# Sin7Y/olavm

Measured on AMD Instinct MI355X. Metric: goldilocks_ntt_throughput, higher is better.
Workload: dtype u64; 1 GPU; batched Goldilocks NTT (cfft::evaluate_poly), 94 cols x 2^22 rows per GPU, resident; log_n=22, columns_per_gpu=94, parallelism=columns sharded over 1 GPU(s), no collective, launch=single process

## Files before the change

olavm_amd/csrc/ntt2.hip:

```cpp
#include <hip/hip_runtime.h>

#include "device_ctx.h"
#include "gl.cuh"
#include "ntt2t.cuh"

namespace ola {

#ifndef NTT2_DEFAULT_GROUP_MB
#define NTT2_DEFAULT_GROUP_MB 0
#endif
#ifndef NTT2_STRIDED_COLS
#define NTT2_STRIDED_COLS 8
#endif

template <int K, bool INV>
__device__ __forceinline__ void dft_pow2(u64* x) {
#pragma unroll
    for (int i = K - 1; i >= 0; --i) {
#pragma unroll
        for (int j = 0; j < (1 << K); ++j) {
            if (j & (1 << i)) continue;
            const int e16 = (j & ((1 << i) - 1)) << (3 - i);
            const int t = ((INV ? 36 : 156) * e16) % 192;
            const u64 a = x[j], c = x[j + (1 << i)];
            x[j] = gl_add(a, c);
            const u64 d = (t >= 96) ? gl_sub(c, a) : gl_sub(a, c);
            x[j + (1 << i)] = gl_mul_pow2_sw(d, t % 96);
        }
    }
}

template <int R, int MODE, bool INV, int CB, bool PRE>
__device__ __forceinline__ void ntt2_pass_body(const Ntt2Params& p) {
    static_assert(!PRE || MODE == N2_STRIDED, "only the first (strided) pass of a coset transform pre-scales");
    static_assert(R >= 4 && R <= 8, "pass width");
    constexpr int K2 = R - 4;
    constexpr int D = 8 - R;
    constexpr int G2 = 1 << K2;
    constexpr int ROW = (1 << R) + 1;
    extern __shared__ __attribute__((aligned(16))) unsigned char smem_raw[];
    u64* lds = reinterpret_cast<u64*>(smem_raw);
    u64* tw1 = lds + ntt2_lds_elems<R, MODE>();

    const int tid = threadIdx.x;
    const u32 blk = blockIdx.x;
    const size_t col0 = (size_t)blockIdx.y * CB, coset = blockIdx.z;
    const int L = p.log_n, lo = p.lo;

    if (R > 4) {
        if (tid < (1 << R)) tw1[tid] = p.tw_r[tid];
    }

    auto pad1 = [](int e) -> int { return K2 >= 1 ? e + ((e >> (K2 + 4)) << 4) : e; };

    int uA, m_low, tA;
    if (MODE == N2_STRIDED) {
        uA = tid & 15;
        const int rest = tid >> 4;
        m_low = rest & ((1 << K2) - 1);
        tA = rest >> K2;
    } else {
        m_low = tid & ((1 << K2) - 1);
        uA = (tid >> K2) & 15;
        tA = tid >> R;
    }
    size_t a0;
    size_t jstride;
    size_t a0_uni = 0;
    u32 a0_lane = 0;
    {
        const u32 ntile = (blk << D) + tA;
        if (MODE == N2_STRIDED) {
            const u32 lowblks = 1u << (lo - 4);
            const u32 lb = ntile & (lowblks - 1), hi = ntile >> (lo - 4);
            a0 = ((size_t)hi << (lo + R)) + ((size_t)lb << 4) + ((size_t)m_low << lo) + uA;
            jstride = (size_t)1 << (lo + K2);
            const u32 ntile0 = blk << D;
            a0_uni = ((size_t)(ntile0 >> (lo - 4)) << (lo + R)) + ((size_t)(ntile0 & (lowblks - 1)) << 4);
            a0_lane = ((u32)tA << 4) + ((u32)m_low << lo) + (u32)uA;
        } else if (MODE == N2_BITREV_LAST) {
            a0 = ((((size_t)ntile << 4) + uA) << R) + m_low;
            jstride = (size_t)1 << K2;
        } else {
            const int ub = L - R - 4;
            const size_t row = ((size_t)rev_bits_c(uA, 4) << ub) + (ub ? bitrev32(ntile, ub) : 0);
            a0 = (row << R) + m_low;
            jstride = (size_t)1 << K2;
        }
    }
    const int uB = tid & 15, m_hi = tid >> 4;

    constexpr bool prescale = PRE;
    u64 up[PRE ? 16 : 1];
    if (prescale) {
        const u64 sb = two_level(p.sc_lo + coset * p.sc_coset_stride, p.sc_hi + coset * p.sc_coset_stride, p.sc_h, a0);
        const u64 st = p.sc_step[coset];
        u64 w = sb;
#pragma unroll
        for (int j = 0; j < 16; j++) {
            up[j] = w;
            if (j < 15) w = gl_mul(w, st);
        }
    }
    u64 wt[16];
    if (MODE == N2_STRIDED) {
        const u32 lowblks = 1u << (lo - 4);
#pragma unroll
        for (int t = 0; t < (1 << D); t++) {
            const u32 ntile = (blk << D) + t;
            const u64 low = ((u64)(ntile & (lowblks - 1)) << 4) + uB;
            u64 base = gl_mul(two_level(p.tw_lo, p.tw_hi, p.tw_h, low * (u64)rev_bits_c(m_hi & 15, 4)), p.post_scale);
            const u64 step = (K2 >= 1) ? two_level(p.tw_lo, p.tw_hi, p.tw_h, low << 4) : 1;
            u64 w = base;
#pragma unroll
            for (int k = 0; k < G2; k++) {
                wt[t * G2 + k] = w;
                if (k + 1 < G2) w = gl_mul(w, step);
            }
        }
    }

#pragma unroll 1
    for (int cc = 0; cc < CB; cc++) {
        const size_t col = col0 + cc;
        if (col >= p.ncols) break;
        const u64* __restrict__ in = p.in + col * p.in_col_stride + coset * p.in_coset_stride;
        u64* __restrict__ out = p.out + col * p.out_col_stride + coset * p.out_coset_stride;
        u32 zlane = 0;
        asm volatile("" : "+v"(zlane));

        {
            u64 x[16];
            if (MODE == N2_STRIDED) {
                const char* __restrict__ base = reinterpret_cast<const char*>(in + a0_uni);
                const u32 off = (a0_lane + zlane) * 8u;
#pragma unroll
                for (int j = 0; j < 16; j++) x[j] = gl_canon(*reinterpret_cast<const u64*>(base + j * jstride * 8 + off));
            } else {
#pragma unroll
                for (int j = 0; j < 16; j++) x[j] = gl_canon(in[a0 + j * jstride]);
            }
            if (prescale) {
#pragma unroll
                for (int j = 0; j < 16; j++) x[j] = gl_mul(x[j], up[j]);
            }
            dft_pow2<4, INV>(x);
            if (R > 4 && cc == 0) __syncthreads();
#pragma unroll
            for (int j = 0; j < 16; j++) {
                const int q1 = rev_bits_c(j, 4);
                u64 v = x[j];
                if (MODE == N2_STRIDED) {
                    if (R > 4 && q1 != 0) v = gl_mul(v, tw1[(q1 << K2) + m_low]);
                } else if (R > 4 && q1 != 0) {
                    const int idx = m_low * q1;
                    if (idx) v = gl_mul(v, tw1[idx]);
                }
                const int m = (j << K2) + m_low;
                if (MODE == N2_STRIDED) lds[pad1((((tA << R) + m) << 4) + uA)] = v;
                else lds[((tA << 4) + uA) * ROW + m] = v;
            }
        }
        __syncthreads();

        {
            u64 y[16];
#pragma unroll
            for (int t = 0; t < (1 << D); t++) {
#pragma unroll
                for (int j2 = 0; j2 < G2; j2++) {
                    const int m = (m_hi << K2) + j2;
                    y[t * G2 + j2] = (MODE == N2_STRIDED) ? lds[pad1((((t << R) + m) << 4) + uB)] : lds[((t << 4) + uB) * ROW + m];
                }
            }
#pragma unroll
            for (int t = 0; t < (1 << D); t++)
                if (K2 >= 1) dft_pow2<(K2 >= 1 ? K2 : 1), INV>(y + t * G2);
            if (MODE == N2_STRIDED) {
                const u32 lowblks = 1u << (lo - 4);
#pragma unroll
                for (int t = 0; t < (1 << D); t++) {
                    const u32 ntile = (blk << D) + t;
                    const u32 lb = ntile & (lowblks - 1), hi = ntile >> (lo - 4);
                    char* __restrict__ obase = reinterpret_cast<char*>(out + ((size_t)hi << (lo + R)) + ((size_t)lb << 4));
                    const u32 ooff = (((u32)m_hi << (K2 + lo)) + (u32)uB + zlane) * 8u;
#pragma unroll
                    for (int k = 0; k < G2; k++) {
                        const int j2 = rev_bits_c(k, K2);
                        *reinterpret_cast<u64*>(obase + ((size_t)j2 << (lo + 3)) + ooff) = gl_mul(y[t * G2 + j2], wt[t * G2 + k]);
                    }
                }
            } else if (MODE == N2_NATURAL_LAST) {
#pragma unroll
                for (int t = 0; t < (1 << D); t++) {
                    const u32 A = (blk << D) + t;
#pragma unroll
                    for (int j2 = 0; j2 < G2; j2++) {
                        const u32 q = ((u32)rev_bits_c(j2, K2) << 4) + (u32)rev_bits_c(m_hi & 15, 4);
                        out[((size_t)A << 4) + uB + ((size_t)q << (L - R))] = y[t * G2 + j2];
                    }
                }
            } else {
                __syncthreads();
#pragma unroll
                for (int t = 0; t < (1 << D); t++)
#pragma unroll
                    for (int j2 = 0; j2 < G2; j2++) lds[((t << 4) + uB) * ROW + (m_hi << K2) + j2] = y[t * G2 + j2];
                __syncthreads();
                const size_t b0 = (size_t)blk << 12;
#pragma unroll
                for (int k = 0; k < 16; k++) {
                    const int c = (k << 8) + tid;
                    out[b0 + c] = lds[(c >> R) * ROW + (c & ((1 << R) - 1))];
                }
            }
        }
        if (cc + 1 < CB) __syncthreads();
    }
}

template <int R, int MODE, bool INV, int CB, bool PRE>
__global__ __launch_bounds__(256) void ntt2_pass_kernel(Ntt2Params p) { ntt2_pass_body<R, MODE, INV, CB, PRE>(p); }
template <int R, int MODE, bool INV, int CB>
static void ntt2_launch_cb(const Ntt2Params& p0, size_t cols, size_t cosets, hipStream_t stream) {
    Ntt2Params p = p0;
    p.ncols = cols;
    const size_t lds_bytes = (size_t)(ntt2_lds_elems<R, MODE>() + (R > 4 ? (1 << R) : 0)) * 8;
    dim3 grid((unsigned)(((size_t)1 << p.log_n) >> 12), (unsigned)((cols + CB - 1) / CB), (unsigned)cosets);
    if (MODE == N2_STRIDED && p.sc_lo) hipLaunchKernelGGL((ntt2_pass_kernel<R, MODE, INV, CB, MODE == N2_STRIDED>), grid, dim3(256), lds_bytes, stream, p);
    else hipLaunchKernelGGL((ntt2_pass_kernel<R, MODE, INV, CB, false>), grid, dim3(256), lds_bytes, stream, p);
}
template <int R, int MODE, bool INV>
static void ntt2_launch(const Ntt2Params& p, size_t cols, size_t cosets, hipStream_t stream) {
    ntt2_launch_cb<R, MODE, INV, (MODE == N2_STRIDED ? NTT2_STRIDED_COLS : 1)>(p, cols, cosets, stream);
}
template <int MODE, bool INV>
static void ntt2_dispatch_r(int R, const Ntt2Params& p, size_t cols, size_t cosets, hipStream_t s) {
    switch (R) {
        case 4: ntt2_launch<4, MODE, INV>(p, cols, cosets, s); break;
        case 5: ntt2_launch<5, MODE, INV>(p, cols, cosets, s); break;
        case 6: ntt2_launch<6, MODE, INV>(p, cols, cosets, s); break;
        case 7: ntt2_launch<7, MODE, INV>(p, cols, cosets, s); break;
        default: ntt2_launch<8, MODE, INV>(p, cols, cosets, s); break;
    }
}
static void ntt2_dispatch(int R, int mode, bool inv, const Ntt2Params& p, size_t cols, size_t cosets, hipStream_t s) {
    if (mode == N2_STRIDED) { if (inv) ntt2_dispatch_r<N2_STRIDED, true>(R, p, cols, cosets, s); else ntt2_dispatch_r<N2_STRIDED, false>(R, p, cols, cosets, s); }
    else if (mode == N2_BITREV_LAST) { if (inv) ntt2_dispatch_r<N2_BITREV_LAST, true>(R, p, cols, cosets, s); else ntt2_dispatch_r<N2_BITREV_LAST, false>(R, p, cols, cosets, s); }
    else { if (inv) ntt2_dispatch_r<N2_NATURAL_LAST, true>(R, p, cols, cosets, s); else ntt2_dispatch_r<N2_NATURAL_LAST, false>(R, p, cols, cosets, s); }
}

static bool ntt2_tform() {
    static const bool v = [] { const char* e = getenv("OLA_NTT2_TFORM"); return !(e && atoi(e) == 0); }();
    return v;
}
template <int R, int MODE, bool INV, int LM>
static void ntt2t_launch(const Ntt2Params& p0, size_t cols, size_t cosets, hipStream_t stream) {
    constexpr int CB = NTT2_STRIDED_COLS;
    Ntt2Params p = p0;
    p.ncols = cols;
    const size_t lds_bytes = (size_t)ntt2_lds_elems<R, MODE>() * 8 + (R > 4 ? ((size_t)sizeof(TfTw) << R) : 0) + (LM == 1 ? ((size_t)8 << R) : 0);
    dim3 grid((unsigned)(((size_t)1 << p.log_n) >> 12), (unsigned)((cols + CB - 1) / CB), (unsigned)cosets);
    hipLaunchKernelGGL((ntt2t_pass_kernel<R, MODE, INV, CB, LM>), grid, dim3(256), lds_bytes, stream, p);
}
template <int MODE, bool INV, int LM>
static void ntt2t_dispatch_r(int R, const Ntt2Params& p, size_t cols, size_t cosets, hipStream_t s) {
    switch (R) {
        case 4: ntt2t_launch<4, MODE, INV, LM>(p, cols, cosets, s); break;
        case 5: ntt2t_launch<5, MODE, INV, LM>(p, cols, cosets, s); break;
        case 6: ntt2t_launch<6, MODE, INV, LM>(p, cols, cosets, s); break;
        case 7: ntt2t_launch<7, MODE, INV, LM>(p, cols, cosets, s); break;
        default: ntt2t_launch<8, MODE, INV, LM>(p, cols, cosets, s); break;
    }
}
template <bool INV>
static void ntt2t_dispatch_inv(int R, int mode, int lm, const Ntt2Params& p, size_t cols, size_t cosets, hipStream_t s) {
    if (mode == N2_STRIDED) {
        if (lm == 0) ntt2t_dispatch_r<N2_STRIDED, INV, 0>(R, p, cols, cosets, s);
        else ntt2t_dispatch_r<N2_STRIDED, INV, 1>(R, p, cols, cosets, s);
    } else if (mode == N2_BITREV_LAST) ntt2t_dispatch_r<N2_BITREV_LAST, INV, 2>(R, p, cols, cosets, s);
    else ntt2t_dispatch_r<N2_NATURAL_LAST, INV, 2>(R, p, cols, cosets, s);
}
static void ntt2t_dispatch(int R, int mode, bool inv, int lm, const Ntt2Params& p, size_t cols, size_t cosets, hipStream_t s) {
    if (inv) ntt2t_dispatch_inv<true>(R, mode, lm, p, cols, cosets, s);
    else ntt2t_dispatch_inv<false>(R, mode, lm, p, cols, cosets, s);
}
static void ntt2t_dispatch_timed(NttTables& t, int R, int mode, bool inv, int lm, const Ntt2Params& p, size_t cols, size_t cosets, hipStream_t s) {
    if (!t.pass_timing || t.pass_recs.size() >= 4096) { ntt2t_dispatch(R, mode, inv, lm, p, cols, cosets, s); return; }
    NttTables::PassRec r{R, mode, lm, inv, ((size_t)1 << p.log_n) * cols * cosets, nullptr, nullptr};
    HIP_CHECK(hipEventCreate(&r.a));
    HIP_CHECK(hipEventCreate(&r.b));
    HIP_CHECK(hipEventRecord(r.a, s));
    ntt2t_dispatch(R, mode, inv, lm, p, cols, cosets, s);
    HIP_CHECK(hipEventRecord(r.b, s));
    t.pass_recs.push_back(r);
}

static const u64* get_round_table(NttTables& t, int R, int inverse) {
    auto key = std::make_pair(200 + R, inverse);
    auto it = t.small.find(key);
    if (it != t.small.end()) return it->second;
    const std::vector<u64> full = powers(root_for(R, inverse), (size_t)1 << R);
    std::vector<u64> v;
    for (int q1 = 0; q1 < 16; q1++)
        for (int m = 0; m < (1 << (R - 4)); m++) v.push_back(full[(size_t)m * q1]);
    return t.small[key] = upload(t.ctx, v);
}

static const u64* get_full_small(NttTables& t, int R, int inverse) {
    auto key = std::make_pair(100 + R, inverse);
    auto it = t.small.find(key);
    if (it != t.small.end()) return it->second;
    std::vector<u64> v = powers(root_for(R, inverse), (size_t)1 << R);
    return t.small[key] = upload(t.ctx, v);
}

static const u64* get_coset_steps(NttTables& t, int log_n, int rate_bits, int e, u64 single_shift) {
    std::vector<u64> v;
    for (u64 s : coset_shifts(log_n, rate_bits, single_shift)) v.push_back(gl_pow(s, (u64)1 << e));
    return upload(t.ctx, v);
}

static const u64* get_coset_pows(NttTables& t, int log_n, int rate_bits, int lo, int R, u64 single_shift) {
    std::vector<u64> v;
    for (u64 sc : coset_shifts(log_n, rate_bits, single_shift)) {
        const std::vector<u64> pw = powers(gl_pow(sc, (u64)1 << lo), (size_t)1 << R);
        v.insert(v.end(), pw.begin(), pw.end());
    }
    return upload(t.ctx, v);
}

static void ntt2_run_group(NttTables& t, const u64* in, size_t in_col_stride, u64* out, size_t out_col_stride, u64* scratch,
                           size_t scratch_col_stride, int L, size_t cols, bool inverse, bool natural_out, int sc_rate_bits, u64 sc_shift,
                           size_t cosets, size_t out_coset_stride, size_t coset_first) {
    hipStream_t stream = t.ctx->stream;
    const int P = (L + 7) / 8;
    std::vector<int> Rs = split_even(L, P);
    std::reverse(Rs.begin(), Rs.end());
    const u64 final_scale = inverse ? gl_inv(((u64)1 << L) % GL_P) : 1;
    u64* work = natural_out ? scratch : out;
    const size_t work_col_stride = natural_out ? scratch_col_stride : out_col_stride;
    const size_t work_coset_stride = natural_out ? 0 : out_coset_stride;

    const u64* cur_in = in;
    size_t cur_in_stride = in_col_stride, cur_in_coset = 0;
    int lo = L;
    if (ntt2_tform() && L <= 28) {
        for (int i = 0; i < P; i++) {
            const int R = Rs[i];
            lo -= R;
            const bool last = (i == P - 1);
            Ntt2Params p = {};
            p.log_n = L; p.lo = lo;
            p.tw_r = get_round_table(t, R, inverse);
            p.post_scale = last ? final_scale : 1;
            p.in = cur_in; p.in_col_stride = cur_in_stride; p.in_coset_stride = cur_in_coset;
            if (i > 0) {
                TwoLevel tw = get_two(t, L - lo, inverse);
                p.tw_lo = tw.lo; p.tw_hi = tw.hi; p.tw_h = tw.h;
            }
            if (sc_rate_bits != -2) {
                const auto skey = std::make_tuple(L, sc_rate_bits, 1000 + lo * 16 + R, sc_rate_bits >= 0 ? (u64)0 : sc_shift);
                auto st = t.coset_steps.find(skey);
                if (st == t.coset_steps.end()) st = t.coset_steps.emplace(skey, get_coset_pows(t, L, sc_rate_bits, lo, R, sc_shift)).first;
                p.sc_pow = st->second + (coset_first << R);
            }
            const int lm = last ? 2 : ((i > 0 || p.sc_pow) ? 1 : 0);
            if (!last) {
                p.out = work; p.out_col_stride = work_col_stride; p.out_coset_stride = work_coset_stride;
                if (lo - 4 < 8 - R) throw OlaError(-7, "ntt2: pass split leaves a strided pass with lo + R < 12");
                ntt2t_dispatch_timed(t, R, N2_STRIDED, inverse, lm, p, cols, cosets, stream);
                cur_in = work; cur_in_stride = work_col_stride; cur_in_coset = work_coset_stride;
            } else {
                p.out = out; p.out_col_stride = out_col_stride; p.out_coset_stride = out_coset_stride;
                ntt2t_dispatch_timed(t, R, natural_out ? N2_NATURAL_LAST : N2_BITREV_LAST, inverse, 2, p, cols, cosets, stream);
            }
        }
        return;
    }
    for (int i = 0; i < P; i++) {
        const int R = Rs[i];
        lo -= R;
        const bool last = (i == P - 1);
        Ntt2Params p = {};
        p.log_n = L; p.lo = lo;
        p.tw_r = last ? get_full_small(t, R, inverse) : get_round_table(t, R, inverse);
        p.post_scale = 1;
        p.in = cur_in; p.in_col_stride = cur_in_stride; p.in_coset_stride = cur_in_coset;
        if (!last) {
            TwoLevel tw = get_two(t, lo + R, inverse);
            p.tw_lo = tw.lo; p.tw_hi = tw.hi; p.tw_h = tw.h;
            if (i == P - 2) p.post_scale = final_scale;
            p.out = work; p.out_col_stride = work_col_stride; p.out_coset_stride = work_coset_stride;
            if (i == 0 && sc_rate_bits != -2) {
                TwoLevel sc;
                size_t stride = 0;
                if (sc_rate_bits >= 0) sc = get_coset(t, L, sc_rate_bits, &stride);
                else sc = get_shift(t, L, sc_shift);
                p.sc_lo = sc.lo + coset_first * stride; p.sc_hi = sc.hi + coset_first * stride; p.sc_h = sc.h; p.sc_coset_stride = stride;
                {
                    const auto skey = std::make_tuple(L, sc_rate_bits, lo + R - 4, sc_rate_bits >= 0 ? (u64)0 : sc_shift);
                    auto st = t.coset_steps.find(skey);
                    if (st == t.coset_steps.end()) st = t.coset_steps.emplace(skey, get_coset_steps(t, L, sc_rate_bits, lo + R - 4, sc_shift)).first;
                    p.sc_step = st->second + coset_first;
                }
            }
            if (lo - 4 < 8 - R) throw OlaError(-7, "ntt2: pass split leaves a strided pass with lo + R < 12");
            ntt2_dispatch(R, N2_STRIDED, inverse, p, cols, cosets, stream);
            cur_in = work; cur_in_stride = work_col_stride; cur_in_coset = work_coset_stride;
        } else {
            p.out = out; p.out_col_stride = out_col_stride; p.out_coset_stride = out_coset_stride;
            ntt2_dispatch(R, natural_out ? N2_NATURAL_LAST : N2_BITREV_LAST, inverse, p, cols, cosets, stream);
        }
    }
}

static size_t ntt2_group_bytes() {
    const char* e = getenv("OLA_NTT2_GROUP_MB");
    return e ? (size_t)atol(e) << 20 : (size_t)NTT2_DEFAULT_GROUP_MB << 20;
}

void ntt2_run(NttTables& t, const u64* in, size_t in_col_stride, u64* out, size_t out_col_stride, u64* scratch,
              size_t scratch_col_stride, int L, size_t cols, bool inverse, bool natural_out, int sc_rate_bits, u64 sc_shift,
              size_t cosets, size_t out_coset_stride, size_t coset_first) {
    if (cols == 0) return;
    const size_t budget = ntt2_group_bytes(), col_bytes = ((size_t)8 << L) * (natural_out ? 2 : 1);
    size_t gc = cols, gk = cosets;
    if (budget && L >= 18 && col_bytes * cols * cosets > budget) {
        const size_t unit = NTT2_STRIDED_COLS;
        gk = 1;
        gc = std::max<size_t>(unit, budget / col_bytes / unit * unit);
        if (gc >= cols) { gc = cols; gk = std::max<size_t>(1, std::min(cosets, budget / (col_bytes * cols))); }
    }
    for (size_t c0 = 0; c0 < cols; c0 += gc) {
        const size_t nc = std::min(gc, cols - c0);
        for (size_t k0 = 0; k0 < cosets; k0 += gk) {
            const size_t nk = std::min(gk, cosets - k0);
            ntt2_run_group(t, in + c0 * in_col_stride, in_col_stride, out + c0 * out_col_stride + k0 * out_coset_stride, out_col_stride,
                           scratch ? scratch + c0 * scratch_col_stride : nullptr, scratch_col_stride, L, nc, inverse, natural_out,
                           sc_rate_bits, sc_shift, nk, out_coset_stride, coset_first + k0);
        }
    }
}

}
```

olavm_amd/csrc/ntt2t.cuh:

```cuda
#pragma once
#include <hip/hip_runtime.h>

#include "gl.cuh"
#include "tform.cuh"

namespace ola {

enum { N2_STRIDED = 0, N2_BITREV_LAST = 1, N2_NATURAL_LAST = 2 };

struct Ntt2Params {
    const u64* in;
    u64* out;
    size_t in_col_stride, out_col_stride, in_coset_stride, out_coset_stride;
    int log_n;
    size_t ncols;
    int lo;
    const u64* tw_r;
    const u64* tw_lo;
    const u64* tw_hi;
    int tw_h;
    u64 post_scale;
    const u64* sc_lo;
    const u64* sc_hi;
    int sc_h;
    size_t sc_coset_stride;
    const u64* sc_step;
    const u64* sc_pow;
};

__device__ __forceinline__ constexpr int rev_bits_c(int x, int bits) {
    int r = 0;
    for (int i = 0; i < bits; i++) r |= ((x >> i) & 1) << (bits - 1 - i);
    return r;
}

__device__ __forceinline__ u64 two_level(const u64* __restrict__ lo, const u64* __restrict__ hi, int h, u64 e) {
    return gl_mul(lo[e & (((u64)1 << h) - 1)], hi[e >> h]);
}

template <int R, int MODE>
constexpr int ntt2_lds_elems() {
    constexpr int K2 = R - 4;
    if (MODE == N2_STRIDED) return 4096 + (K2 >= 1 ? 16 * (4096 >> (K2 + 4)) : 0);
    return (1 << (8 - R)) * 16 * ((1 << R) + 1);
}

template <int R, int MODE, bool INV, int CB, int LM>
__device__ __forceinline__ void ntt2t_pass_body(const Ntt2Params& p) {
    static_assert(R >= 4 && R <= 8, "pass width");
    static_assert((LM == 2) == (MODE != N2_STRIDED), "strided passes keep their multipliers in LDS, closing passes in registers");
    constexpr int K2 = R - 4;
    constexpr int D = 8 - R;
    constexpr int G2 = 1 << K2;
    constexpr int ROW = (1 << R) + 1;
    extern __shared__ __attribute__((aligned(16))) unsigned char smem_raw[];
    u64* lds = reinterpret_cast<u64*>(smem_raw);
    TfTw* tw1 = reinterpret_cast<TfTw*>(lds + ntt2_lds_elems<R, MODE>());
    u64* lmtab = reinterpret_cast<u64*>(tw1 + (R > 4 ? (1 << R) : 0));

    const int tid = threadIdx.x;
    const u32 blk = blockIdx.x;
    const size_t col0 = (size_t)blockIdx.y * CB, coset = blockIdx.z;
    const int L = p.log_n, lo = p.lo;

    if (R > 4) {
        if (tid < (1 << R)) tw1[tid] = tf_split_u64(p.tw_r[tid]);
    }

    auto pad1 = [](int e) -> int { return K2 >= 1 ? e + ((e >> (K2 + 4)) << 4) : e; };

    int uA, m_low, tA;
    if (MODE == N2_STRIDED) {
        uA = tid & 15;
        const int rest = tid >> 4;
        m_low = rest & ((1 << K2) - 1);
        tA = rest >> K2;
    } else {
        m_low = tid & ((1 << K2) - 1);
        uA = (tid >> K2) & 15;
        tA = tid >> R;
    }
    size_t a0, jstride;
    size_t a0_uni = 0;
    u32 a0_lane = 0;
    {
        const u32 ntile = (blk << D) + tA;
        if (MODE == N2_STRIDED) {
            const u32 lowblks = 1u << (lo - 4);
            const u32 lb = ntile & (lowblks - 1), hi = ntile >> (lo - 4);
            a0 = ((size_t)hi << (lo + R)) + ((size_t)lb << 4) + ((size_t)m_low << lo) + uA;
            jstride = (size_t)1 << (lo + K2);
            const u32 ntile0 = blk << D;
            a0_uni = ((size_t)(ntile0 >> (lo - 4)) << (lo + R)) + ((size_t)(ntile0 & (lowblks - 1)) << 4);
            a0_lane = ((u32)tA << 4) + ((u32)m_low << lo) + (u32)uA;
        } else if (MODE == N2_BITREV_LAST) {
            a0 = ((((size_t)ntile << 4) + uA) << R) + m_low;
            jstride = (size_t)1 << K2;
        } else {
            const int ub = L - R - 4;
            const size_t row = ((size_t)rev_bits_c(uA, 4) << ub) + (ub ? bitrev32(ntile, ub) : 0);
            a0 = (row << R) + m_low;
            jstride = (size_t)1 << K2;
        }
    }
    const int uB = tid & 15, m_hi = tid >> 4;

    const int HB = L - lo - R;
    u64 wl[LM == 2 ? 16 : 1];
    if (LM == 1) {
        if (tid < (1 << R)) {
            const u32 hi = (blk << D) >> (lo - 4);
            const u64 K = HB ? bitrev32(hi, HB) : 0;
            u64 v = 1;
            if (p.tw_lo) v = two_level(p.tw_lo, p.tw_hi, p.tw_h, K * (u64)tid);
            if (p.sc_pow) v = p.tw_lo ? gl_mul(v, p.sc_pow[(coset << R) + tid]) : p.sc_pow[(coset << R) + tid];
            lmtab[tid] = v;
        }
    } else if (LM == 2) {
        const u64 K = bitrev32((u32)(a0 >> R), HB);
        u64 base = gl_mul(two_level(p.tw_lo, p.tw_hi, p.tw_h, K * (u64)m_low), p.post_scale);
        u64 step = two_level(p.tw_lo, p.tw_hi, p.tw_h, K << K2);
        if (p.sc_pow) {
            base = gl_mul(base, p.sc_pow[(coset << R) + m_low]);
            step = gl_mul(step, p.sc_pow[(coset << R) + (1 << K2)]);
        }
        u64 w = base;
#pragma unroll
        for (int j = 0; j < 16; j++) {
            wl[j] = w;
            if (j < 15) w = gl_mul(w, step);
        }
    }

    if (LM == 1 || R > 4) __syncthreads();

#pragma unroll 1
    for (int cc = 0; cc < CB; cc++) {
        const size_t col = col0 + cc;
        if (col >= p.ncols) break;
        const u64* __restrict__ in = p.in + col * p.in_col_stride + coset * p.in_coset_stride;
        u64* __restrict__ out = p.out + col * p.out_col_stride + coset * p.out_coset_stride;
        u32 zlane = 0;
        asm volatile("" : "+v"(zlane));

        T4 y[16];
        {
            T4 x[16];
            {
                u64 raw[16];
                if (MODE == N2_STRIDED) {
                    const char* __restrict__ base = reinterpret_cast<const char*>(in + a0_uni);
                    const u32 off = (a0_lane + zlane) * 8u;
#pragma unroll
                    for (int j = 0; j < 16; j++) raw[j] = *reinterpret_cast<const u64*>(base + j * jstride * 8 + off);
                } else {
#pragma unroll
                    for (int j = 0; j < 16; j++) raw[j] = in[a0 + j * jstride];
                }
#pragma unroll
                for (int j = 0; j < 16; j++) {
                    if (LM) {
                        u64 plo, phi;
                        mul_wide(raw[j], LM == 1 ? lmtab[(j << K2) + m_low] : wl[j], plo, phi);
                        x[j] = tf_from_u128(plo, phi);
                    } else {
                        x[j] = tf_from_u64(raw[j]);
                    }
                }
            }
            tf_dft<4, INV>(x);
            if (R > 4) {
#pragma unroll
                for (int j = 0; j < 16; j++) {
                    const int q1 = rev_bits_c(j, 4);
                    if (q1 != 0) x[j] = tf_mul(x[j], tw1[(q1 << K2) + m_low]);
                    else x[j] = tf_norm(x[j]);
                }
            }
#pragma unroll
            for (int h = 0; h < 2; h++) {
                if (h == 1) __syncthreads();
#pragma unroll
                for (int j = 0; j < 16; j++) {
                    const int m = (j << K2) + m_low;
                    const u64 v = (u64)(u32)x[j].v[2 * h] | ((u64)(u32)x[j].v[2 * h + 1] << 32);
                    if (MODE == N2_STRIDED) lds[pad1((((tA << R) + m) << 4) + uA)] = v;
                    else lds[((tA << 4) + uA) * ROW + m] = v;
                }
                __syncthreads();
#pragma unroll
                for (int t = 0; t < (1 << D); t++) {
#pragma unroll
                    for (int j2 = 0; j2 < G2; j2++) {
                        const int m = (m_hi << K2) + j2;
                        const u64 v = (MODE == N2_STRIDED) ? lds[pad1((((t << R) + m) << 4) + uB)] : lds[((t << 4) + uB) * ROW + m];
                        y[t * G2 + j2].v[2 * h] = (i32)(u32)v;
                        y[t * G2 + j2].v[2 * h + 1] = (i32)(u32)(v >> 32);
                    }
                }
            }
        }

#pragma unroll
        for (int t = 0; t < (1 << D); t++)
            if (K2 >= 1) tf_dft<(K2 >= 1 ? K2 : 1), INV>(y + t * G2);
        if (MODE == N2_STRIDED) {
            const u32 lowblks = 1u << (lo - 4);
#pragma unroll
            for (int t = 0; t < (1 << D); t++) {
                const u32 ntile = (blk << D) + t;
                const u32 lb = ntile & (lowblks - 1), hi = ntile >> (lo - 4);
                char* __restrict__ obase = reinterpret_cast<char*>(out + ((size_t)hi << (lo + R)) + ((size_t)lb << 4));
                const u32 ooff = (((u32)m_hi << (K2 + lo)) + (u32)uB + zlane) * 8u;
#pragma unroll
                for (int j2 = 0; j2 < G2; j2++)
                    *reinterpret_cast<u64*>(obase + ((size_t)j2 << (lo + 3)) + ooff) = tf_to_u64<false>(y[t * G2 + j2]);
            }
        } else if (MODE == N2_NATURAL_LAST) {
#pragma unroll
            for (int t = 0; t < (1 << D); t++) {
                const u32 A = (blk << D) + t;
                const u32 ooff = ((((u32)rev_bits_c(m_hi & 15, 4)) << (L - R)) + (u32)uB + zlane) * 8u;
#pragma unroll
                for (int j2 = 0; j2 < G2; j2++) {
                    char* __restrict__ obase = reinterpret_cast<char*>(out + ((size_t)A << 4) + ((size_t)rev_bits_c(j2, K2) << (L - R + 4)));
                    *reinterpret_cast<u64*>(obase + ooff) = tf_to_u64<true>(y[t * G2 + j2]);
                }
            }
        } else {
            __syncthreads();
#pragma unroll
            for (int t = 0; t < (1 << D); t++)
#pragma unroll
                for (int j2 = 0; j2 < G2; j2++) lds[((t << 4) + uB) * ROW + (m_hi << K2) + j2] = tf_to_u64<true>(y[t * G2 + j2]);
            __syncthreads();
            const size_t b0 = (size_t)blk << 12;
#pragma unroll
            for (int k = 0; k < 16; k++) {
                const int c = (k << 8) + tid;
                out[b0 + c] = lds[(c >> R) * ROW + (c & ((1 << R) - 1))];
            }
        }
        if (cc + 1 < CB) __syncthreads();
    }
}

template <int R, int MODE, bool INV, int CB, int LM>
__global__ __launch_bounds__(256, (MODE == N2_STRIDED ? 4 : 1)) void ntt2t_pass_kernel(Ntt2Params p) { ntt2t_pass_body<R, MODE, INV, CB, LM>(p); }

}
```

olavm_amd/csrc/tform.cuh:

```cuda
#pragma once
#include "gl.cuh"

namespace ola {

typedef int i32;
typedef long long i64;

GL_HD u32 tf_alignbit(u32 hi, u32 lo, int s) {
#if defined(__HIP_DEVICE_COMPILE__)
    return __builtin_amdgcn_alignbit(hi, lo, s);
#else
    return (u32)((((u64)hi << 32) | lo) >> s);
#endif
}

struct T4 {
    i32 v[4];
};
struct TfTw {
    i32 w0, w1, w2, pad;
};

GL_HD void tf_pin(T4& y) {
#if defined(__HIP_DEVICE_COMPILE__)
    asm("" : "+v"(y.v[0]), "+v"(y.v[1]), "+v"(y.v[2]), "+v"(y.v[3]));
#else
    (void)y;
#endif
}

GL_HD TfTw tf_split_u64(u64 w) {
    const u32 lo = (u32)w, hi = (u32)(w >> 32);
    TfTw t;
    t.w0 = (i32)(lo & 0xFFFFFFu);
    t.w1 = (i32)(((lo >> 24) | (hi << 8)) & 0xFFFFFFu);
    t.w2 = (i32)(hi >> 16);
    t.pad = 0;
    return t;
}

GL_HD T4 tf_from_u64(u64 x) {
    const u32 lo = (u32)x, hi = (u32)(x >> 32);
    T4 r;
    r.v[0] = (i32)(lo & 0xFFFFFFu);
    r.v[1] = (i32)(tf_alignbit(hi, lo, 24) & 0xFFFFFFu);
    r.v[2] = (i32)(hi >> 16);
    r.v[3] = 0;
    return r;
}
GL_HD T4 tf_from_u128(u64 lo, u64 hi) {
    const u32 l0 = (u32)lo, l1 = (u32)(lo >> 32), h0 = (u32)hi, h1 = (u32)(hi >> 32);
    T4 r;
    r.v[0] = (i32)(l0 & 0xFFFFFFu) - (i32)(h1 & 0xFFFFFFu);
    r.v[1] = (i32)(tf_alignbit(l1, l0, 24) & 0xFFFFFFu) - (i32)(h1 >> 24);
    r.v[2] = (i32)(tf_alignbit(h0, l1, 16) & 0xFFFFFFu);
    r.v[3] = (i32)(h0 >> 8);
    return r;
}

template <bool CANON>
GL_HD u64 tf_to_u64(const T4& x) {
    u32 u0 = (u32)x.v[0] + 0x80000080u, u1 = (u32)x.v[1] + 0x7FFFFF80u;
    u32 u2 = (u32)x.v[2] + 0x7FFFFF80u, u3 = (u32)x.v[3] + 0x7FFFFF80u;
    const u32 n1 = u1 & 0xFFFFFFu;
    u2 += u1 >> 24;
    const u32 n2 = u2 & 0xFFFFFFu;
    u3 += u2 >> 24;
    const u32 n3 = u3 & 0xFFFFFFu;
    u0 -= u3 >> 24;
    const u64 A = (u64)n1 * 0x1000000ull + u0;
    const u32 chi = (n3 << 8) | (n2 >> 16);
    const u32 d16 = n2 << 16;
#if defined(OLA_GL_ASM)
    const u32 a_lo = (u32)A, a_hi = (u32)(A >> 32);
    u32 hi1, e1, e2;
    u64 cA, cB, t2;
    asm("v_add_co_u32_e64 %0, %1, %2, %3" : "=v"(hi1), "=s"(cA) : "v"(a_hi), "v"(d16));
    asm("s_nop 1\n\tv_cndmask_b32_e64 %0, 0, -1, %1" : "=v"(e1) : "s"(cA));
    const u64 lo = (((u64)hi1 << 32) | a_lo) + e1;
    asm("v_mad_u64_u32 %0, %1, %2, -1, %3" : "=v"(t2), "=s"(cB) : "v"(chi), "v"(lo));
    if (!CANON) {
        asm("s_nop 1\n\tv_cndmask_b32_e64 %0, 0, -1, %1" : "=v"(e2) : "s"(cB));
        return t2 + e2;
    }
    const u32 tl = (u32)t2, th = (u32)(t2 >> 32);
    u32 ul, uh, r0, r1;
    u64 c1, c2, m;
    asm("v_add_co_u32_e64 %0, %1, -1, %2" : "=v"(ul), "=s"(c1) : "v"(tl));
    asm("s_nop 1\n\tv_addc_co_u32_e64 %0, %1, 0, %2, %3" : "=v"(uh), "=s"(c2) : "v"(th), "s"(c1));
    asm("s_nop 1\n\ts_or_b64 %2, %3, %4\n\tv_cndmask_b32_e64 %0, %5, %6, %2\n\tv_cndmask_b32_e64 %1, %7, %8, %2"
        : "=&v"(r0), "=&v"(r1), "=&s"(m) : "s"(cB), "s"(c2), "v"(tl), "v"(ul), "v"(th), "v"(uh) : "scc");
    return ((u64)r1 << 32) | r0;
#else
    u64 lo = A + ((u64)d16 << 32);
    if (lo < A) lo += GL_EPS;
    const u64 prod = (u64)chi * GL_EPS;
    u64 t2 = lo + prod;
    if (t2 < lo) t2 += GL_EPS;
    return CANON ? gl_canon(t2) : t2;
#endif
}

GL_HD T4 tf_add(const T4& a, const T4& b) {
    T4 r;
#pragma unroll
    for (int i = 0; i < 4; i++) r.v[i] = a.v[i] + b.v[i];
    return r;
}

GL_HD T4 tf_norm(const T4& x) {
    const i32 mask = 0xFFFFFF;
    T4 y;
    y.v[0] = (x.v[0] & mask) - (x.v[3] >> 24);
    y.v[1] = (x.v[1] & mask) + (x.v[0] >> 24);
    y.v[2] = (x.v[2] & mask) + (x.v[1] >> 24);
    y.v[3] = (x.v[3] & mask) + (x.v[2] >> 24);
    return y;
}

template <int S>
GL_HD T4 tf_sub_mul_pow2(const T4& a, const T4& b) {
    static_assert(S >= 0 && S < 192, "shift out of range");
    constexpr int q8 = S / 24, r = S % 24, q = q8 & 3;
    constexpr bool neg = q8 >= 4;
    T4 o;
    if (r == 0) {
#pragma unroll
        for (int i = 0; i < 4; i++) {
            const bool flip = neg != (i + q >= 4);
            o.v[(i + q) & 3] = flip ? (b.v[i] - a.v[i]) : (a.v[i] - b.v[i]);
        }
    } else {
        constexpr int k = 24 - r;
        const i32 mask = (i32)((1 << k) - 1);
        T4 d;
#pragma unroll
        for (int i = 0; i < 4; i++) d.v[i] = neg ? (b.v[i] - a.v[i]) : (a.v[i] - b.v[i]);
        T4 y;
        y.v[0] = ((d.v[0] & mask) << r) - (d.v[3] >> k);
        y.v[1] = ((d.v[1] & mask) << r) + (d.v[0] >> k);
        y.v[2] = ((d.v[2] & mask) << r) + (d.v[1] >> k);
        y.v[3] = ((d.v[3] & mask) << r) + (d.v[2] >> k);
#pragma unroll
        for (int i = 0; i < 4; i++) {
            if (i + q >= 4) o.v[(i + q) & 3] = -y.v[i];
            else o.v[i + q] = y.v[i];
        }
    }
    return o;
}

GL_HD T4 tf_mul(const T4& x_in, const TfTw& w) {
    T4 x = x_in;
    tf_pin(x);
    const i32 w0 = w.w0, w1 = w.w1, w2 = w.w2;
    const i32 n2 = -x.v[2], n3 = -x.v[3];
    i64 z[4];
    z[0] = (i64)x.v[0] * w0 + (i64)n3 * w1 + (i64)n2 * w2;
    z[1] = (i64)x.v[0] * w1 + (i64)x.v[1] * w0 + (i64)n3 * w2;
    z[2] = (i64)x.v[0] * w2 + (i64)x.v[1] * w1 + (i64)x.v[2] * w0;
    z[3] = (i64)x.v[1] * w2 + (i64)x.v[2] * w1 + (i64)x.v[3] * w0;
    i32 l[4], m[4], h[4];
#pragma unroll
    for (int k = 0; k < 4; k++) {
        const u32 lo = (u32)(u64)z[k];
        const i32 hi = (i32)(z[k] >> 32);
        l[k] = (i32)(lo & 0xFFFFFFu);
        m[k] = (i32)(tf_alignbit((u32)hi, lo, 24) & 0xFFFFFFu);
        h[k] = hi >> 16;
    }
    T4 y;
    y.v[0] = l[0] - m[3] - h[2];
    y.v[1] = l[1] + m[0] - h[3];
    y.v[2] = l[2] + m[1] + h[0];
    y.v[3] = l[3] + m[2] + h[1];
    tf_pin(y);
    return y;
}

GL_HD constexpr int tf_root_exp(int k, bool inv) {
    int e = 39;
    for (int i = k; i < 6; i++) e = (2 * e) % 192;
    return inv ? (192 - e) % 192 : e;
}

template <int K, bool INV>
GL_HD void tf_dft(T4* x) {
    static_assert(K >= 0 && K <= 4, "radix");
#pragma unroll
    for (int i = K - 1; i >= 0; --i) {
#pragma unroll
        for (int j = 0; j < (1 << K); ++j) {
            if (j & (1 << i)) continue;
            const int e = (j & ((1 << i) - 1)) << (3 - i);
            const int s = (tf_root_exp(4, INV) * e) % 192;
            const T4 a = x[j], b = x[j + (1 << i)];
            x[j] = tf_add(a, b);
            switch (s) {
#define OLA_TF_CASE(S) case S: x[j + (1 << i)] = tf_sub_mul_pow2<S>(a, b); break;
                OLA_TF_CASE(0) OLA_TF_CASE(12) OLA_TF_CASE(24) OLA_TF_CASE(36) OLA_TF_CASE(48) OLA_TF_CASE(60) OLA_TF_CASE(72) OLA_TF_CASE(84)
                OLA_TF_CASE(96) OLA_TF_CASE(108) OLA_TF_CASE(120) OLA_TF_CASE(132) OLA_TF_CASE(144) OLA_TF_CASE(156) OLA_TF_CASE(168)
                OLA_TF_CASE(180)
#undef OLA_TF_CASE
                default: break;
            }
        }
    }
}

}
```

Measured before the change: 1510 GB/s.

## Close Goldilocks NTT with a 6-bit pass using shift-only twiddles

```diff
diff --git a/olavm_amd/csrc/ntt2.hip b/olavm_amd/csrc/ntt2.hip
--- a/olavm_amd/csrc/ntt2.hip
+++ b/olavm_amd/csrc/ntt2.hip
@@ -254,12 +254,32 @@
     static const bool v = [] { const char* e = getenv("OLA_NTT2_TFORM"); return !(e && atoi(e) == 0); }();
     return v;
 }
+static int ntt2_close6() {
+    static const int v = [] { const char* e = getenv("OLA_NTT2_CLOSE6"); return e ? atoi(e) : 1; }();
+    return v;
+}
+static std::vector<int> ntt2t_widths(int L) {
+    const int P = (L + 7) / 8;
+    std::vector<int> even = split_even(L, P);
+    std::reverse(even.begin(), even.end());
+    if (ntt2_close6() == 0 || (P < 3 && ntt2_close6() != 2)) return even;
+    std::vector<int> v = split_even(L - 6, P - 1);
+    std::reverse(v.begin(), v.end());
+    int lo = L;
+    for (int R : v) {
+        lo -= R;
+        if (R < 4 || R > 8 || lo - 4 < 8 - R) return even;
+    }
+    v.push_back(6);
+    return v;
+}
 template <int R, int MODE, bool INV, int LM>
 static void ntt2t_launch(const Ntt2Params& p0, size_t cols, size_t cosets, hipStream_t stream) {
     constexpr int CB = NTT2_STRIDED_COLS;
     Ntt2Params p = p0;
     p.ncols = cols;
-    const size_t lds_bytes = (size_t)ntt2_lds_elems<R, MODE>() * 8 + (R > 4 ? ((size_t)sizeof(TfTw) << R) : 0) + (LM == 1 ? ((size_t)8 << R) : 0);
+    constexpr bool tw1 = R > 4 && !(R == 6 && MODE != N2_STRIDED);
+    const size_t lds_bytes = (size_t)ntt2_lds_elems<R, MODE>() * 8 + (tw1 ? ((size_t)sizeof(TfTw) << R) : 0) + (LM == 1 ? ((size_t)8 << R) : 0);
     dim3 grid((unsigned)(((size_t)1 << p.log_n) >> 12), (unsigned)((cols + CB - 1) / CB), (unsigned)cosets);
     hipLaunchKernelGGL((ntt2t_pass_kernel<R, MODE, INV, CB, LM>), grid, dim3(256), lds_bytes, stream, p);
 }
@@ -346,6 +366,7 @@
     size_t cur_in_stride = in_col_stride, cur_in_coset = 0;
     int lo = L;
     if (ntt2_tform() && L <= 28) {
+        Rs = ntt2t_widths(L);
         for (int i = 0; i < P; i++) {
             const int R = Rs[i];
             lo -= R;
diff --git a/olavm_amd/csrc/ntt2t.cuh b/olavm_amd/csrc/ntt2t.cuh
--- a/olavm_amd/csrc/ntt2t.cuh
+++ b/olavm_amd/csrc/ntt2t.cuh
@@ -45,6 +45,12 @@
     return (1 << (8 - R)) * 16 * ((1 << R) + 1);
 }
 
+template <int ML, bool INV>
+__device__ __forceinline__ void ntt2t_close6_put(const T4* x, int h, u64* dst) {
+    if (h == 0) tf_round6_pair<ML, INV, 0>(x, dst, 4);
+    else tf_round6_pair<ML, INV, 1>(x, dst, 4);
+}
+
 template <int R, int MODE, bool INV, int CB, int LM>
 __device__ __forceinline__ void ntt2t_pass_body(const Ntt2Params& p) {
     static_assert(R >= 4 && R <= 8, "pass width");
@@ -53,6 +59,7 @@
     constexpr int D = 8 - R;
     constexpr int G2 = 1 << K2;
     constexpr int ROW = (1 << R) + 1;
+    constexpr bool CLOSE6 = (R == 6 && MODE != N2_STRIDED);
     extern __shared__ __attribute__((aligned(16))) unsigned char smem_raw[];
     u64* lds = reinterpret_cast<u64*>(smem_raw);
     TfTw* tw1 = reinterpret_cast<TfTw*>(lds + ntt2_lds_elems<R, MODE>());
@@ -63,7 +70,7 @@
     const size_t col0 = (size_t)blockIdx.y * CB, coset = blockIdx.z;
     const int L = p.log_n, lo = p.lo;
 
-    if (R > 4) {
+    if (R > 4 && !CLOSE6) {
         if (tid < (1 << R)) tw1[tid] = tf_split_u64(p.tw_r[tid]);
     }
 
@@ -75,6 +82,10 @@
         const int rest = tid >> 4;
         m_low = rest & ((1 << K2) - 1);
         tA = rest >> K2;
+    } else if (CLOSE6) {
+        m_low = __builtin_amdgcn_readfirstlane(tid >> 6);
+        uA = tid & 15;
+        tA = (tid >> 4) & 3;
     } else {
         m_low = tid & ((1 << K2) - 1);
         uA = (tid >> K2) & 15;
@@ -132,7 +143,7 @@
         }
     }
 
-    if (LM == 1 || R > 4) __syncthreads();
+    if (LM == 1 || (R > 4 && !CLOSE6)) __syncthreads();
 
 #pragma unroll 1
     for (int cc = 0; cc < CB; cc++) {
@@ -153,6 +164,22 @@
                     const u32 off = (a0_lane + zlane) * 8u;
 #pragma unroll
                     for (int j = 0; j < 16; j++) raw[j] = *reinterpret_cast<const u64*>(base + j * jstride * 8 + off);
+                } else if (CLOSE6) {
+                    const u32 wv = (u32)m_low, ln = (u32)tid & 63u;
+                    const u32 ntile = (blk << D) + wv;
+                    const u32 off = (ln + zlane) * 8u;
+#pragma unroll
+                    for (int k = 0; k < 16; k++) {
+                        size_t row;
+                        if (MODE == N2_BITREV_LAST) row = ((size_t)ntile << 4) + k;
+                        else row = ((size_t)rev_bits_c(k, 4) << (L - R - 4)) + bitrev32(ntile, L - R - 4);
+                        raw[k] = *reinterpret_cast<const u64*>(reinterpret_cast<const char*>(in + (row << R)) + off);
+                    }
+#pragma unroll
+                    for (int k = 0; k < 16; k++) lds[((wv << 4) + k) * ROW + ln] = raw[k];
+                    __syncthreads();
+#pragma unroll
+                    for (int j = 0; j < 16; j++) raw[j] = lds[((tA << 4) + uA) * ROW + (j << K2) + m_low];
                 } else {
 #pragma unroll
                     for (int j = 0; j < 16; j++) raw[j] = in[a0 + j * jstride];
@@ -169,7 +196,11 @@
                 }
             }
             tf_dft<4, INV>(x);
-            if (R > 4) {
+            if (CLOSE6) {
+#pragma unroll
+                for (int j = 0; j < 16; j++) tf_pin(x[j]);
+            }
+            if (R > 4 && !CLOSE6) {
 #pragma unroll
                 for (int j = 0; j < 16; j++) {
                     const int q1 = rev_bits_c(j, 4);
@@ -179,9 +210,18 @@
             }
 #pragma unroll
             for (int h = 0; h < 2; h++) {
-                if (h == 1) __syncthreads();
-#pragma unroll
-                for (int j = 0; j < 16; j++) {
+                if (h == 1 || CLOSE6) __syncthreads();
+                if (CLOSE6) {
+                    u64* dst = lds + ((tA << 4) + uA) * ROW + m_low;
+                    switch (m_low) {
+                        case 0: ntt2t_close6_put<0, INV>(x, h, dst); break;
+                        case 1: ntt2t_close6_put<1, INV>(x, h, dst); break;
+                        case 2: ntt2t_close6_put<2, INV>(x, h, dst); break;
+                        default: ntt2t_close6_put<3, INV>(x, h, dst); break;
+                    }
+                }
+#pragma unroll
+                for (int j = 0; j < 16 && !CLOSE6; j++) {
                     const int m = (j << K2) + m_low;
                     const u64 v = (u64)(u32)x[j].v[2 * h] | ((u64)(u32)x[j].v[2 * h + 1] << 32);
                     if (MODE == N2_STRIDED) lds[pad1((((tA << R) + m) << 4) + uA)] = v;
diff --git a/olavm_amd/csrc/tform.cuh b/olavm_amd/csrc/tform.cuh
--- a/olavm_amd/csrc/tform.cuh
+++ b/olavm_amd/csrc/tform.cuh
@@ -14,8 +14,14 @@
 #endif
 }
 
+#if defined(OLA_TF_LIMB)
+typedef OLA_TF_LIMB tf_limb;
+#else
+typedef i32 tf_limb;
+#endif
+
 struct T4 {
-    i32 v[4];
+    tf_limb v[4];
 };
 struct TfTw {
     i32 w0, w1, w2, pad;
@@ -150,11 +156,36 @@
     return o;
 }
 
+template <int S, int T>
+GL_HD tf_limb tf_mul_pow2_limb(const T4& x) {
+    static_assert(S >= 0 && S < 192 && T >= 0 && T < 4, "shift or limb out of range");
+    constexpr int q8 = S / 24, r = S % 24, q = q8 & 3;
+    constexpr int i = (T - q) & 3;
+    constexpr bool flip = (q8 >= 4) != (i + q >= 4);
+    tf_limb y = x.v[i];
+    if (r != 0) {
+        constexpr int k = 24 - r;
+        const i32 mask = (i32)((1 << k) - 1);
+        const tf_limb lo = (x.v[i] & mask) << r, hi = x.v[(i + 3) & 3] >> k;
+        y = (i == 0) ? lo - hi : lo + hi;
+    }
+    return flip ? -y : y;
+}
+template <int S>
+GL_HD T4 tf_mul_pow2(const T4& x) {
+    T4 o;
+    o.v[0] = tf_mul_pow2_limb<S, 0>(x);
+    o.v[1] = tf_mul_pow2_limb<S, 1>(x);
+    o.v[2] = tf_mul_pow2_limb<S, 2>(x);
+    o.v[3] = tf_mul_pow2_limb<S, 3>(x);
+    return o;
+}
+
 GL_HD T4 tf_mul(const T4& x_in, const TfTw& w) {
     T4 x = x_in;
     tf_pin(x);
     const i32 w0 = w.w0, w1 = w.w1, w2 = w.w2;
-    const i32 n2 = -x.v[2], n3 = -x.v[3];
+    const tf_limb n2 = -x.v[2], n3 = -x.v[3];
     i64 z[4];
     z[0] = (i64)x.v[0] * w0 + (i64)n3 * w1 + (i64)n2 * w2;
     z[1] = (i64)x.v[0] * w1 + (i64)x.v[1] * w0 + (i64)n3 * w2;
@@ -182,6 +213,27 @@
     int e = 39;
     for (int i = k; i < 6; i++) e = (2 * e) % 192;
     return inv ? (192 - e) % 192 : e;
+}
+
+GL_HD void tf_pin2(tf_limb& a, tf_limb& b) {
+#if defined(__HIP_DEVICE_COMPILE__)
+    asm("" : "+v"(a), "+v"(b));
+#else
+    (void)a;
+    (void)b;
+#endif
+}
+template <int ML, bool INV, int H, int J = 0>
+GL_HD void tf_round6_pair(const T4* x, u64* out, int stride) {
+    static_assert(ML >= 0 && ML < 4 && (H == 0 || H == 1), "second-round index of a 6-bit pass, half of the limbs");
+    if constexpr (J < 16) {
+        constexpr int q1 = ((J & 1) << 3) | ((J & 2) << 1) | ((J & 4) >> 1) | ((J & 8) >> 3);
+        constexpr int S = (tf_root_exp(6, INV) * ML * q1) % 192;
+        tf_limb a = tf_mul_pow2_limb<S, 2 * H>(x[J]), b = tf_mul_pow2_limb<S, 2 * H + 1>(x[J]);
+        tf_pin2(a, b);
+        out[J * stride] = (u64)(u32)a | ((u64)(u32)b << 32);
+        tf_round6_pair<ML, INV, H, J + 1>(x, out, stride);
+    }
 }
 
 template <int K, bool INV>
```

Result: faster. 1547 GB/s (median of 6 runs) (+2.4%).
